# 0xC0000054/pdn-jpegxl

Measured on AMD Instinct MI355X. Metric: megapixels/sec decode (4K lossy VarDCT), higher is better.
Workload: dtype f32

## Files before the change

### pdn_jpegxl_amd/csrc/tile_kernels.hip

```cpp
#include <hip/hip_runtime.h>
#include <cstdlib>
#include "dev_types.h"
#include "dev_util.h"
#include "kernels.h"

namespace jxlhip {

#ifndef JXLHIP_PRIO_PIXEL
#define JXLHIP_PRIO_PIXEL 0
#endif
#if JXLHIP_PRIO_PIXEL
#define JXL_PIXEL_PRIO() __builtin_amdgcn_s_setprio(JXLHIP_PRIO_PIXEL)
#else
#define JXL_PIXEL_PRIO() ((void)0)
#endif

namespace {

constexpr int kTS = 64;
constexpr int kLP = 65;

__device__ const uint8_t t_quant_table[kNumStrategies] = {0, 1, 2, 3, 4, 5, 6, 6, 7, 7, 8, 8, 9, 9, 10, 10, 10, 10, 11, 12, 12, 13, 14, 14, 15, 16, 16};

__device__ __forceinline__ bool Special(uint32_t s) { return (s >= 1 && s <= 3) || (s >= 12 && s <= 17); }
typedef float __attribute__((ext_vector_type(4))) F4;
template <int N>
__device__ __forceinline__ F4 MfmaChain(const float* pa, int sa, const float* pb, int sb) {
  float a[N / 4], b[N / 4];
#pragma unroll
  for (int k = 0; k < N / 4; k++) { a[k] = pa[k * sa]; b[k] = pb[k * sb]; }
  F4 acc = {0.f, 0.f, 0.f, 0.f};
#pragma unroll
  for (int k = 0; k < N / 4; k++) acc = __builtin_amdgcn_mfma_f32_16x16x4f32(a[k], b[k], acc, 0, 0, 0);
  return acc;
}
template <bool kTableIsA>
__device__ __forceinline__ F4 MfmaChain32L(const float4* t_lo, const float4* t_hi, int pair, const float* po, int so) {
  const float4 v0 = t_lo[pair], v1 = t_hi[pair];
  const float t[8] = {v0.x, v0.y, v0.z, v0.w, v1.x, v1.y, v1.z, v1.w};
  float o[8];
#pragma unroll
  for (int k = 0; k < 8; k++) o[k] = po[k * so];
  F4 acc = {0.f, 0.f, 0.f, 0.f};
#pragma unroll
  for (int k = 0; k < 8; k++)
    acc = kTableIsA ? __builtin_amdgcn_mfma_f32_16x16x4f32(t[k], o[k], acc, 0, 0, 0) : __builtin_amdgcn_mfma_f32_16x16x4f32(o[k], t[k], acc, 0, 0, 0);
  return acc;
}
template <bool kTableIsA>
__device__ __forceinline__ F4 MfmaChain64L(const float4* t64, int pair, const float* po, int so) {
  float t[16], o[16];
#pragma unroll
  for (int j = 0; j < 4; j++) {
    const float4 v = t64[j * 256 + pair];
    t[4 * j] = v.x; t[4 * j + 1] = v.y; t[4 * j + 2] = v.z; t[4 * j + 3] = v.w;
  }
#pragma unroll
  for (int k = 0; k < 16; k++) o[k] = po[k * so];
  F4 acc = {0.f, 0.f, 0.f, 0.f};
#pragma unroll
  for (int k = 0; k < 16; k++)
    acc = kTableIsA ? __builtin_amdgcn_mfma_f32_16x16x4f32(t[k], o[k], acc, 0, 0, 0) : __builtin_amdgcn_mfma_f32_16x16x4f32(o[k], t[k], acc, 0, 0, 0);
  return acc;
}
__device__ __forceinline__ bool MfmaRows(uint32_t tl, uint32_t tr) {
  return (tl >> 31) && (tr >> 31) && ((tl >> 21) & 7) >= 1 && ((tl >> 21) & 7) == ((tr >> 21) & 7) && ((tl >> 13) & 31) == ((tr >> 13) & 31);
}
__device__ __forceinline__ bool MfmaCols(uint32_t tl, uint32_t bl) {
  return (tl >> 31) && (bl >> 31) && ((tl >> 18) & 7) >= 1 && ((tl >> 18) & 7) == ((bl >> 18) & 7) && ((tl >> 8) & 31) == ((bl >> 8) & 31);
}

__device__ __forceinline__ float SrgbOetfT(float v) {
  const float lin = 12.92f * v;
  const float cur = 1.055f * __builtin_amdgcn_exp2f(__builtin_amdgcn_logf(v) * (1.0f / 2.4f)) - 0.055f;
  return v <= 0.0031308f ? lin : cur;
}
__device__ __forceinline__ float SrgbOetf255T(float v) {
  const float lin = (12.92f * 255.0f) * v;
  const float cur = (1.055f * 255.0f) * __builtin_amdgcn_exp2f(__builtin_amdgcn_logf(v) * (1.0f / 2.4f)) - (0.055f * 255.0f);
  return v <= 0.0031308f ? lin : cur;
}
__device__ __forceinline__ float PowT(float a, float e) { return __builtin_amdgcn_exp2f(__builtin_amdgcn_logf(a) * e); }
__device__ __forceinline__ float EncodeTransferT(int kind, float v, float pq_scale, const float* lut = nullptr) {
  if (kind == 0) return v;
  if (kind == 5) {
    const float t = __builtin_sqrtf(fminf(fmaxf(v, 0.f), 1.f)) * 4095.0f;
    const int i = min((int)t, 4094);
    return lut[i] + (lut[i + 1] - lut[i]) * (t - (float)i);
  }
  const float a = fabsf(v);
  float r;
  if (kind == 1) r = a <= 0.0031308f ? 12.92f * a : 1.055f * PowT(a, 1.0f / 2.4f) - 0.055f;
  else if (kind == 2) r = a < 0.018f ? 4.5f * a : 1.099f * PowT(a, 0.45f) - 0.099f;
  else {
    const float xp = a > 0.f ? PowT(a * pq_scale, 0.1593017578125f) : 0.f;
    r = a > 0.f ? PowT((0.8359375f + 18.8515625f * xp) / (1.0f + 18.6875f * xp), 78.84375f) : 0.f;
  }
  return copysignf(r, v);
}
__device__ __forceinline__ uint8_t ToU8T(float v) {
  v = fminf(fmaxf(v * 255.0f, 0.f), 255.0f);
  return (uint8_t)(v + 0.5f);
}

__device__ __forceinline__ uint32_t LoadAlpha(const DevImage& im, size_t i) {
// ... 44 lines not shown
    }
  }
}
__device__ __forceinline__ void WritePixelA(const DevImage& im, int x, int y, float X, float Y, float B, uint32_t a) {
  WritePixelAt(im, [&] { return (size_t)(y - im.band_y0) * im.w + x; }, X, Y, B, a);
}
__device__ __forceinline__ bool PlainOutput(const DevImage& im) { return im.out_bits == 8 && im.to_srgb <= 1 && !im.unpremultiply && !im.has_noise; }
__device__ __forceinline__ float NoiseStrength(const DevImage& im, float v) {
  const float s = fmaxf(0.f, 6.0f * v);
  const int i = (int)fminf(s, 6.0f);
  const float t = fminf(s - (float)i, 1.0f);
  const float lo = im.noise_lut[i], hi = im.noise_lut[i + 1];
  return fminf(fmaxf(lo + (hi - lo) * t, 0.f), 1.0f);
}
__device__ __forceinline__ void AddNoise(const DevImage& im, int x, int y, float& X, float& Y, float& B) {
  const size_t o = (size_t)y * im.w + x;
  const float n0 = im.noise[0][o], n1 = im.noise[1][o], n2 = im.noise[2][o];
  const float sr = NoiseStrength(im, 0.5f * (Y + X)), sg = NoiseStrength(im, 0.5f * (Y - X));
  const float shared = n2 * (127.0f / 128.0f);
  const float red = (n0 * (1.0f / 128.0f) + shared) * sr, green = (n1 * (1.0f / 128.0f) + shared) * sg;
  const float rg = red + green;
  X += im.base_x * rg + (red - green);
  Y += rg;
  B += im.base_b * rg;
}
__device__ __forceinline__ uint32_t PixelToRgba8(const DevImage& im, float X, float Y, float B, uint32_t a) {
  const float gr = Y + X - im.opsin_bias_cbrt[0], gg = Y - X - im.opsin_bias_cbrt[1], gb = B - im.opsin_bias_cbrt[2];
  const float mr = gr * gr * gr + im.opsin_bias[0], mg = gg * gg * gg + im.opsin_bias[1], mb = gb * gb * gb + im.opsin_bias[2];
  float r = im.opsin_inv[0] * mr + im.opsin_inv[1] * mg + im.opsin_inv[2] * mb;
  float g = im.opsin_inv[3] * mr + im.opsin_inv[4] * mg + im.opsin_inv[5] * mb;
  float bl = im.opsin_inv[6] * mr + im.opsin_inv[7] * mg + im.opsin_inv[8] * mb;
  if (im.to_srgb) { r = SrgbOetf255T(r); g = SrgbOetf255T(g); bl = SrgbOetf255T(bl); }
  else { r *= 255.0f; g *= 255.0f; bl *= 255.0f; }
  uint32_t px = a << 24;
  px = __builtin_amdgcn_cvt_pk_u8_f32(r, 0, px);
  px = __builtin_amdgcn_cvt_pk_u8_f32(g, 1, px);
  px = __builtin_amdgcn_cvt_pk_u8_f32(bl, 2, px);
  return px;
}
__device__ __noinline__ void WritePixelGeneral(const DevImage& im, int x, int y, float X, float Y, float B, uint32_t a) {
  if (im.has_noise) {
    AddNoise(im, x, y, X, Y, B);
    if (im.out_bits == 8 && im.to_srgb <= 1 && !im.unpremultiply && im.final_stage == 5 &&
        (im.noise_pairs_twin || (im.nch_out == 4 && (x | 3) < im.w))) {
      const uint32_t px = PixelToRgba8(im, X, Y, B, a);
      uint8_t* out = im.out + ((size_t)(y - im.band_y0) * im.w + x) * im.nch_out;
      if (im.nch_out == 4) *(uint32_t*)out = px;
      else if (im.nch_out == 3) { out[0] = (uint8_t)px; out[1] = (uint8_t)(px >> 8); out[2] = (uint8_t)(px >> 16); }
      else { out[0] = (uint8_t)(px >> 8); if (im.nch_out == 2) out[1] = (uint8_t)(px >> 24); }
      return;
    }
  }
  WritePixelA(im, x, y, X, Y, B, a);
}
__device__ __forceinline__ void WritePixel(const DevImage& im, int x, int y, float X, float Y, float B) {
  const uint32_t a = im.has_alpha ? LoadAlpha(im, (size_t)y * im.w + x) : 0u;
  if (im.has_noise) { WritePixelGeneral(im, x, y, X, Y, B, a); return; }
  WritePixelA(im, x, y, X, Y, B, a);
}

}

#define JXL_IDCT_STEP(Bp, v0, v1)                                                                  \
  {                                                                                                \
    const float4 b0 = *(const float4*)(Bp);                                                        \
    const float4 b1 = *(const float4*)((Bp) + 4);                                                  \
    a0[0] += v0 * b0.x; a0[1] += v0 * b0.y; a0[2] += v0 * b0.z; a0[3] += v0 * b0.w;                \
    a0[4] += v0 * b1.x; a0[5] += v0 * b1.y; a0[6] += v0 * b1.z; a0[7] += v0 * b1.w;                \
    a1[0] += v1 * b0.x; a1[1] += v1 * b0.y; a1[2] += v1 * b0.z; a1[3] += v1 * b0.w;                \
    a1[4] += v1 * b1.x; a1[5] += v1 * b1.y; a1[6] += v1 * b1.z; a1[7] += v1 * b1.w;                \
  }

__device__ __forceinline__ float DequantBias(int32_t v, float qb, float qb3) {
  if (v == 0) return 0.f;
  if (v == 1) return qb;
  if (v == -1) return -qb;
  const float f = (float)v;
  return f - qb3 * __builtin_amdgcn_rcpf(f);
}
typedef int __attribute__((ext_vector_type(4))) I4v;

constexpr int kTileF = kTS * kLP;

__global__ __launch_bounds__(768, 6) void recon_tile_kernel(const DevImage* __restrict__ imgs, const float* basis_all, const float* basis_small,
                                                             const float* llf_scale, const float* basis_mfma) {
  JXL_PIXEL_PRIO();
  extern __shared__ __align__(16) uint8_t smem_raw[];
  float* cfc3 = (float*)smem_raw;
  float* B816 = cfc3 + 3 * kTileF;
  float* cscale = B816 + 320;
  uint32_t* ci = (uint32_t*)(cscale + 64);
  uint32_t* cmeta = ci + 64;
  uint32_t* cnq = cmeta + 64;
  uint32_t* cpre = cnq + 64;
  uint32_t* cstart = cpre + 3 * 64;
  uint32_t* ctot = cstart + 3 * 64;
  const U32x2** csc = (const U32x2**)(ctot + 4);
  float4* t32_lo = (float4*)(csc + 64);
  float4* t32_hi = t32_lo + 128;
  float4* t64 = t32_hi + 128;
  const DevImage& im = imgs[blockIdx.y];
  const int tile = blockIdx.x;
  if (tile >= im.wt * im.ht) return;
  const int tid = threadIdx.x;
  const int tx = tile % im.wt, ty = tile / im.wt;
  if (ty < im.dec_gy0 * 4 || ty >= im.dec_gy1 * 4) return;
  const int wave = tid >> 6, lane = tid & 63, team = wave >> 2, tw = wave & 3;
  const int c = team == 0 ? 1 : (team == 1 ? 0 : 2);
  const int wp = im.wp, hp = im.hp;
  {
    float4* z = (float4*)cfc3;
    for (int i = tid; i < 3 * kTileF / 4; i += 768) z[i] = make_float4(0.f, 0.f, 0.f, 0.f);
  }
  int bad = 0, has64 = 0;
  if (tid < 64) {
    const int cx = tx * 8 + (tid & 7), cy = ty * 8 + (tid >> 3);
    const bool inside = cx < im.w8 && cy < im.h8;
    const size_t cell_g = (size_t)min(cy, im.h8 - 1) * im.w8 + min(cx, im.w8 - 1);
    const size_t ncells = (size_t)im.w8 * im.h8;
    const uint32_t info_g = im.cellinfo[cell_g];
    const uint32_t rq_g = im.rawq[cell_g];
    U32x2 blk[3];
    blk[0] = im.cblk[ncells + cell_g]; blk[1] = im.cblk[cell_g]; blk[2] = im.cblk[2 * ncells + cell_g];
    const uint32_t info = inside ? info_g : 0u;
    const uint32_t rqv = inside ? rq_g : 1u;
    const int ix = (info >> 8) & 31, iy = (info >> 13) & 31, lcx = (info >> 18) & 7, lcy = (info >> 21) & 7;
    if (inside) {
      if (!(info >> 31)) bad = 1;
      else {
        const int ox = (tid & 7) - ix, oy = (tid >> 3) - iy;
        bad = ox < 0 || oy < 0 || ox + (1 << lcx) > 8 || oy + (1 << lcy) > 8 || Special(info & 0xFF) ||
              (ox & ((1 << lcx) - 1)) != 0 || (oy & ((1 << lcy) - 1)) != 0;
      }
    }
    const bool valid = (info >> 31) && !bad;
    has64 = valid && (lcx == 3 || lcy == 3);
    {
      const uint64_t any = __ballot(has64);
      if (tid == 0) ctot[3] = any != 0;
    }
    const uint32_t q = t_quant_table[valid ? (info & 0xFF) : 0];
    const uint32_t rq_origin = (uint32_t)__shfl((int)rqv, valid ? tid - iy * 8 - ix : tid);
    const uint32_t lng = 3 + max(lcx, lcy);
    const bool transposed = lcy >= lcx;
    ci[tid] = info;
    cscale[tid] = im.inv_global_scale / (float)rq_origin;
    cmeta[tid] = lng | (transposed ? 16u : 0u);
    cnq[tid] = im.dq_n[q];
    csc[tid] = im.scan[q];
    const bool origin = valid && ix == 0 && iy == 0;
    uint32_t cnt[3], sum[3];
#pragma unroll
    for (int t = 0; t < 3; t++) {
      cnt[t] = origin ? blk[t].y : 0u;
      if (cnt[t] > 65536u || blk[t].x > kGroupEntriesCap - cnt[t]) cnt[t] = 0;
      sum[t] = cnt[t];
    }
#pragma unroll
    for (int d = 1; d < 64; d <<= 1) {
#pragma unroll
      for (int t = 0; t < 3; t++) {
        const uint32_t a = (uint32_t)__shfl_up((int)sum[t], d);
        if (tid >= d) sum[t] += a;
      }
    }
#pragma unroll
    for (int t = 0; t < 3; t++) {
      cpre[t * 64 + tid] = sum[t] - cnt[t];
      cstart[t * 64 + tid] = blk[t].x;
      if (tid == 63) ctot[t] = sum[t];
    }
  } else if (tid < 64 + 320) {
    B816[tid - 64] = basis_all[tid - 64];
  } else if (tid < 64 + 320 + 256) {
    const int i = tid - (64 + 320);
    const float4 v = ((const float4*)basis_mfma)[i];
    if (i & 1) t32_hi[i >> 1] = v; else t32_lo[i >> 1] = v;
  }
  if (im.num_passes > 1) bad = 1;
  if (__syncthreads_or(bad)) {
    if (tid == 0) im.tile_list[atomicAdd(&im.status[1], 1u)] = (uint32_t)tile;
    return;
  }
  if (ctot[3]) {
    for (int i = tid; i < 1024; i += 768) t64[(i & 3) * 256 + (i >> 2)] = ((const float4*)(basis_mfma + 1024))[i];
  }
  const float* const Bl = basis_all;
  float* const cfc = cfc3 + team * kTileF;
  if (tw == 0) {
    const int cxg = tx * 8 + (lane & 7), cyg = ty * 8 + (lane >> 3);
    const bool inside = cxg < im.w8 && cyg < im.h8;
    const float lf_g = im.lf_final[c][(size_t)min(cyg, im.h8 - 1) * im.w8 + min(cxg, im.w8 - 1)];
    const float lfv = inside ? lf_g : 0.f;
    const uint32_t info = ci[lane];
    const bool valid = info >> 31;
    const int ix = (info >> 8) & 31, iy = (info >> 13) & 31, lcx = (info >> 18) & 7, lcy = (info >> 21) & 7;
    const int cx = 1 << lcx, cy = 1 << lcy;
    const int ox = (lane & 7) - ix, oy = (lane >> 3) - iy;
    const float* Bx = basis_small + (cx * cx - 1) / 3 + ix * cx;
    const float* By = basis_small + (cy * cy - 1) / 3 + iy * cy;
    float bx[8], byv[8];
#pragma unroll
    for (int k = 0; k < 8; k++) { bx[k] = (valid && k < cx) ? Bx[k] : 0.f; byv[k] = (valid && k < cy) ? By[k] : 0.f; }
    const float sc = valid ? llf_scale[lcy * 32 + iy] * llf_scale[lcx * 32 + ix] / (float)(cx * cy) : 0.f;
    float row = 0.f;
#pragma unroll
    for (int k = 0; k < 8; k++) {
      const float v = __shfl(lfv, (lane - ix + k) & 63);
      if (valid && k < cx) row += v * bx[k];
    }
    float acc = 0.f;
#pragma unroll
    for (int k = 0; k < 8; k++) {
      const float v = __shfl(row, ((oy + k) * 8 + (lane & 7)) & 63);
      if (valid && k < cy) acc += v * byv[k];
    }
    if (valid) atomicAdd(&cfc[(oy * 8 + iy) * kLP + ox * 8 + ix], acc * sc);
  }
  {
    const size_t tile_cfl = (size_t)ty * im.wt + tx;
    const float cfl_x = im.base_x + (float)im.ytox[tile_cfl] * im.inv_color_factor;
    const float cfl_b = im.base_b + (float)im.ytob[tile_cfl] * im.inv_color_factor;
    const uint32_t* entries = im.centries + (size_t)((ty >> 2) * im.xg + (tx >> 2) - im.centries_g0) * kGroupEntriesCap;
    const uint32_t t0 = ctot[0], t01 = t0 + ctot[1], total = t01 + ctot[2];
    const float qb3 = im.qbias[3];
    for (uint32_t e = (uint32_t)tid; e < total; e += 768) {
      const uint32_t t = (e >= t0) + (e >= t01);
      const uint32_t el = e - (t == 0 ? 0u : (t == 1 ? t0 : t01));
      const uint32_t* pre = cpre + t * 64;
      uint32_t j = 0;
#pragma unroll
      for (int step = 32; step; step >>= 1) if (pre[j + step] <= el) j += step;
      const uint32_t ent = entries[cstart[t * 64 + j] + (el - pre[j])];
      const uint32_t k = ent & 0xFFFFu, nq = cnq[j];
      if (k >= nq) continue;
      const int chan = t == 0 ? 1 : (t == 1 ? 0 : 2);
      const U32x2 se = csc[j][(size_t)chan * nq + k];
      const uint32_t meta = cmeta[j];
      const uint32_t lng = meta & 15, p = se.x;
      const uint32_t r = p >> lng, cc = p & ((1u << lng) - 1);
      const uint32_t ky = (meta & 16) ? cc : r, kx = (meta & 16) ? r : cc;
      if (ky >= 64 || kx >= 64) continue;
      const int32_t v = (int32_t)ent >> 16;
      const float dm = t == 0 ? 1.0f : (t == 1 ? im.x_dm : im.b_dm);
      const float o = DequantBias(v, im.qbias[chan], qb3) * (cscale[j] * dm) * __uint_as_float(se.y);
      const uint32_t at = ((j >> 3) * 8 + ky) * kLP + (j & 7) * 8 + kx;
      atomicAdd(&cfc3[t * kTileF + at], o);
      if (t == 0) {
        if (cfl_x != 0.f) atomicAdd(&cfc3[kTileF + at], o * cfl_x);
        if (cfl_b != 0.f) atomicAdd(&cfc3[2 * kTileF + at], o * cfl_b);
      }
    }
  }
  __syncthreads();
  const int l16 = tid & 15, lq = lane >> 4;
  {
    F4 acc[4];
    bool m[4];
    const int x0 = tw * 16;
#pragma unroll
    for (int rb = 0; rb < 4; rb++) {
      const uint32_t inf = ci[rb * 16 + tw * 2];
      m[rb] = MfmaRows(inf, ci[rb * 16 + tw * 2 + 1]);
      if (m[rb]) {
        const int iy = (inf >> 13) & 31, lcy = (inf >> 21) & 7, R = 8 << lcy;
        const float* cp = cfc + ((rb * 2 - iy) * 8 + lq) * kLP + x0 + l16;
        if (R == 16) acc[rb] = MfmaChain<16>(B816 + 64 + lq * 16 + iy * 8 + l16, 64, cp, 4 * kLP);
        else if (R == 32) acc[rb] = MfmaChain32L<true>(t32_lo, t32_hi, (iy * 8 + l16) * 4 + lq, cp, 4 * kLP);
        else acc[rb] = MfmaChain64L<true>(t64, (iy * 8 + l16) * 4 + lq, cp, 4 * kLP);
      }
    }
    const int x = x0 + (lane & 7) * 2, cr = lane >> 3;
    const uint32_t info = ci[cr * 8 + (x >> 3)];
    const bool valu = (info >> 31) && !MfmaRows(ci[(cr >> 1) * 16 + (x >> 4) * 2], ci[(cr >> 1) * 16 + (x >> 4) * 2 + 1]);
    float a0[8] = {0, 0, 0, 0, 0, 0, 0, 0}, a1[8] = {0, 0, 0, 0, 0, 0, 0, 0};
    if (valu) {
      const int iy = (info >> 13) & 31, lcy = (info >> 21) & 7;
      const int R = 8 << lcy;
      const float* in = cfc + (cr - iy) * 8 * kLP + x;
      if (R == 8) {
#pragma unroll 2
        for (int k = 0; k < 8; k++) { const float v0 = in[k * kLP], v1 = in[k * kLP + 1]; JXL_IDCT_STEP(B816 + k * 8, v0, v1) }
      } else if (R == 16) {
        const float* B = B816 + 64 + iy * 8;
#pragma unroll 2
        for (int k = 0; k < 16; k++) { const float v0 = in[k * kLP], v1 = in[k * kLP + 1]; JXL_IDCT_STEP(B + k * 16, v0, v1) }
      } else {
        const float* B = Bl + (R * R - 64) / 3 + iy * 8;
        for (int k = 0; k < R; k++) { const float v0 = in[k * kLP], v1 = in[k * kLP + 1]; JXL_IDCT_STEP(B + k * R, v0, v1) }
      }
    }
    __builtin_amdgcn_fence(__ATOMIC_RELEASE, "wavefront");
    __builtin_amdgcn_wave_barrier();
#pragma unroll
    for (int rb = 0; rb < 4; rb++)
      if (m[rb]) {
        float* o = cfc + (rb * 16 + 4 * lq) * kLP + x0 + l16;
        o[0] = acc[rb].x; o[kLP] = acc[rb].y; o[2 * kLP] = acc[rb].z; o[3 * kLP] = acc[rb].w;
      }
    if (valu) {
#pragma unroll
      for (int j = 0; j < 8; j++) { cfc[(cr * 8 + j) * kLP + x] = a0[j]; cfc[(cr * 8 + j) * kLP + x + 1] = a1[j]; }
    }
  }
  __syncthreads();
  {
    F4 acc[4];
    bool m[4];
    const int y0 = tw * 16;
#pragma unroll
    for (int cs = 0; cs < 4; cs++) {
      const uint32_t inf = ci[tw * 16 + cs * 2];
      m[cs] = MfmaCols(inf, ci[tw * 16 + 8 + cs * 2]);
      if (m[cs]) {
        const int ix = (inf >> 8) & 31, lcx = (inf >> 18) & 7, C = 8 << lcx;
        const float* ap = cfc + (y0 + l16) * kLP + (cs * 2 - ix) * 8 + lq;
        if (C == 16) acc[cs] = MfmaChain<16>(ap, 4, B816 + 64 + lq * 16 + ix * 8 + l16, 64);
        else if (C == 32) acc[cs] = MfmaChain32L<false>(t32_lo, t32_hi, (ix * 8 + l16) * 4 + lq, ap, 4);
        else acc[cs] = MfmaChain64L<false>(t64, (ix * 8 + l16) * 4 + lq, ap, 4);
      }
    }
    const int y = y0 + (lane & 7) * 2, cc = lane >> 3;
    const uint32_t info = ci[(y >> 3) * 8 + cc];
    const bool valu = (info >> 31) && !MfmaCols(ci[(y >> 4) * 16 + (cc >> 1) * 2], ci[(y >> 4) * 16 + 8 + (cc >> 1) * 2]);
    float a0[8] = {0, 0, 0, 0, 0, 0, 0, 0}, a1[8] = {0, 0, 0, 0, 0, 0, 0, 0};
    if (valu) {
      const int ix = (info >> 8) & 31, lcx = (info >> 18) & 7;
      const int C = 8 << lcx;
      const float* in = cfc + y * kLP + (cc - ix) * 8;
      if (C == 8) {
#pragma unroll 2
        for (int k = 0; k < 8; k++) { const float v0 = in[k], v1 = in[k + kLP]; JXL_IDCT_STEP(B816 + k * 8, v0, v1) }
      } else if (C == 16) {
        const float* B = B816 + 64 + ix * 8;
#pragma unroll 2
        for (int k = 0; k < 16; k++) { const float v0 = in[k], v1 = in[k + kLP]; JXL_IDCT_STEP(B + k * 16, v0, v1) }
      } else {
        const float* B = Bl + (C * C - 64) / 3 + ix * 8;
        for (int k = 0; k < C; k++) { const float v0 = in[k], v1 = in[k + kLP]; JXL_IDCT_STEP(B + k * C, v0, v1) }
      }
    }
    __builtin_amdgcn_fence(__ATOMIC_RELEASE, "wavefront");
    __builtin_amdgcn_wave_barrier();
#pragma unroll
    for (int cs = 0; cs < 4; cs++)
      if (m[cs]) {
        float* o = cfc + (y0 + 4 * lq) * kLP + cs * 16 + l16;
        o[0] = acc[cs].x; o[kLP] = acc[cs].y; o[2 * kLP] = acc[cs].z; o[3 * kLP] = acc[cs].w;
      }
    if (valu) {
#pragma unroll
      for (int j = 0; j < 8; j++) { cfc[y * kLP + cc * 8 + j] = a0[j]; cfc[(y + 1) * kLP + cc * 8 + j] = a1[j]; }
    }
    __builtin_amdgcn_fence(__ATOMIC_ACQ_REL, "wavefront");
    __builtin_amdgcn_wave_barrier();
    float* dst = im.xyb[c];
    const int x4 = l16 * 4;
    const int gx = tx * kTS + x4;
#pragma unroll
    for (int it = 0; it < 4; it++) {
      const int yl = y0 + lq + 4 * it;
      const int gy = ty * kTS + yl;
      const float* r = cfc + yl * kLP + x4;
      const float4 o = make_float4(r[0], r[1], r[2], r[3]);
      if (gx < wp && gy < hp) *(float4*)(dst + (size_t)gy * wp + gx) = o;
    }
  }
}

template <int kStage>
__global__ __launch_bounds__(256) void filter_tile_kernel(const DevImage* __restrict__ imgs) {
  JXL_PIXEL_PRIO();
  constexpr int TW = 64, TH = 32;
  constexpr int HALO = kStage == 0 ? 1 : (kStage == 1 ? 3 : (kStage == 2 ? 2 : 1));
  constexpr int LW = TW + 2 * HALO, LH = TH + 2 * HALO;
  __shared__ float t[3][LH][LW + 1];
  const DevImage& im = imgs[blockIdx.y];
  if (!im.stage_on[kStage]) return;
  const int w = im.w, h = im.h, wp = im.wp;
  const int tiles_x = (w + TW - 1) / TW, tiles_y = (h + TH - 1) / TH;
  if ((int)blockIdx.x >= tiles_x * tiles_y) return;
  const int tx = blockIdx.x % tiles_x, ty = blockIdx.x / tiles_x;
  const int x0 = tx * TW, y0 = ty * TH;
  const bool final_stage = im.final_stage == kStage;
  const int row_lo = final_stage ? im.band_y0 : max(0, im.band_y0 - 8), row_hi = final_stage ? im.band_y1 : min(h, im.band_y1 + 8);
  if (y0 + TH <= row_lo || y0 >= row_hi) return;
  const float* in0 = im.stage_in[kStage][0];
  const float* in1 = im.stage_in[kStage][1];
  const float* in2 = im.stage_in[kStage][2];
  constexpr int kLoadIters = (LW * LH + 255) / 256;
#pragma unroll
  for (int it = 0; it < kLoadIters; it++) {
    const int e0 = threadIdx.x + it * 256;
    const int e = e0 < LW * LH ? e0 : LW * LH - 1;
    const int ly = e / LW, lx = e % LW;
    const size_t g = (size_t)ReflectIndex(y0 - HALO + ly, h) * wp + ReflectIndex(x0 - HALO + lx, w);
    const float v0 = in0[g], v1 = in1[g], v2 = in2[g];
    t[0][ly][lx] = v0;
    t[1][ly][lx] = v1;
    t[2][ly][lx] = v2;
  }
  __syncthreads();
#pragma unroll 2
  for (int e = threadIdx.x; e < TW * TH; e += 256) {
    const int ly = e / TW, lx = e % TW;
    const int x = x0 + lx, y = y0 + ly;
    if (x >= w || y < row_lo || y >= row_hi) continue;
    const int cy = ly + HALO, cx = lx + HALO;
    float o0, o1, o2;
    if (kStage == 0) {
      float o[3];
#pragma unroll
      for (int c = 0; c < 3; c++) {
        o[c] = t[c][cy][cx] * im.gab_w[c][0] +
               (t[c][cy - 1][cx] + t[c][cy + 1][cx] + t[c][cy][cx - 1] + t[c][cy][cx + 1]) * im.gab_w[c][1] +
               (t[c][cy - 1][cx - 1] + t[c][cy - 1][cx + 1] + t[c][cy + 1][cx - 1] + t[c][cy + 1][cx + 1]) * im.gab_w[c][2];
      }
      o0 = o[0]; o1 = o[1]; o2 = o[2];
    } else {
      constexpr int kNoff = kStage == 1 ? 12 : 4;
      constexpr int kNplus = kStage == 3 ? 1 : 5;
      const int off0[12][2] = {{-2, 0}, {-1, -1}, {-1, 0}, {-1, 1}, {0, -2}, {0, -1}, {0, 1}, {0, 2}, {1, -1}, {1, 0}, {1, 1}, {2, 0}};
      const int off1[4][2] = {{-1, 0}, {0, -1}, {0, 1}, {1, 0}};
      const int plus[5][2] = {{0, 0}, {-1, 0}, {1, 0}, {0, -1}, {0, 1}};
      const float is = im.inv_sigma[(size_t)(y >> 3) * im.w8 + (x >> 3)];
      o0 = t[0][cy][cx]; o1 = t[1][cy][cx]; o2 = t[2][cy][cx];
      if (!(is < -3.90524291751269967465540850526868f)) {
        const float sm = kStage == 1 ? im.epf_pass0_sigma_scale : (kStage == 2 ? 1.0f : im.epf_pass2_sigma_scale);
        const bool border = ((x & 7) == 0) || ((x & 7) == 7) || ((y & 7) == 0) || ((y & 7) == 7);
        const float inv = is * (border ? sm * im.epf_border_sad_mul : sm);
        float wsum = 1.0f;
#pragma unroll
        for (int k = 0; k < kNoff; k++) {
          const int dy = kStage == 1 ? off0[k][0] : off1[k][0], dx = kStage == 1 ? off0[k][1] : off1[k][1];
          float s0 = 0.f, s1 = 0.f, s2 = 0.f;
#pragma unroll
          for (int p = 0; p < kNplus; p++) {
            const int ay = cy + plus[p][0], ax = cx + plus[p][1];
            s0 += fabsf(t[0][ay][ax] - t[0][ay + dy][ax + dx]);
            s1 += fabsf(t[1][ay][ax] - t[1][ay + dy][ax + dx]);
            s2 += fabsf(t[2][ay][ax] - t[2][ay + dy][ax + dx]);
          }
          const float sad = s0 * im.epf_channel_scale[0] + s1 * im.epf_channel_scale[1] + s2 * im.epf_channel_scale[2];
          const float wt = fmaxf(0.0f, 1.0f + sad * inv);
          wsum += wt;
          o0 += wt * t[0][cy + dy][cx + dx];
          o1 += wt * t[1][cy + dy][cx + dx];
          o2 += wt * t[2][cy + dy][cx + dx];
        }
        const float iw = 1.0f / wsum;
        o0 *= iw; o1 *= iw; o2 *= iw;
      }
    }
    if (final_stage) {
      WritePixel(im, x, y, o0, o1, o2);
    } else {
      const size_t g = (size_t)y * wp + x;
      im.stage_out[kStage][0][g] = o0;
      im.stage_out[kStage][1][g] = o1;
      im.stage_out[kStage][2][g] = o2;
    }
  }
}

constexpr int kStripLanes = 64;
constexpr int kStripOut = 4 * (kStripLanes - 2);
constexpr int kGroupsPerWg = 256 / kStripLanes;
constexpr int kSegRows = 128;
__device__ __forceinline__ float DppFromLeft(float v) {
  return __builtin_bit_cast(float, __builtin_amdgcn_update_dpp(0, __builtin_bit_cast(int, v), 0x138 , 0xF, 0xF, true));
}
__device__ __forceinline__ float DppFromRight(float v) {
  return __builtin_bit_cast(float, __builtin_amdgcn_update_dpp(0, __builtin_bit_cast(int, v), 0x130 , 0xF, 0xF, true));
}
__device__ __forceinline__ F4 ShiftFromLeft(F4 v) { return F4{DppFromLeft(v.w), v.x, v.y, v.z}; }
__device__ __forceinline__ F4 ShiftFromRight(F4 v) { return F4{v.y, v.z, v.w, DppFromRight(v.x)}; }
__device__ __forceinline__ F4 ShiftFromLeft2(F4 v) { return F4{DppFromLeft(v.z), DppFromLeft(v.w), v.x, v.y}; }
__device__ __forceinline__ F4 Abs(F4 v) { return F4{fabsf(v.x), fabsf(v.y), fabsf(v.z), fabsf(v.w)}; }
typedef float __attribute__((ext_vector_type(2))) F2;
typedef unsigned __attribute__((ext_vector_type(2))) U2v;
__device__ __forceinline__ F2 ShiftFromLeft(F2 v) { return F2{DppFromLeft(v.y), v.x}; }
__device__ __forceinline__ F2 ShiftFromRight(F2 v) { return F2{v.y, DppFromRight(v.x)}; }
__device__ __forceinline__ F2 ShiftFromLeft2(F2 v) { return F2{DppFromLeft(v.x), DppFromLeft(v.y)}; }
__device__ __forceinline__ F2 Abs(F2 v) { return F2{fabsf(v.x), fabsf(v.y)}; }

template <typename V> struct RowOf { V c[3]; };
template <typename V> constexpr int kLanePixels = sizeof(V) / sizeof(float);
typedef RowOf<F4> Row3;
typedef RowOf<F2> PairRow;
#define JXL_GLOBAL __attribute__((address_space(1)))
__device__ __forceinline__ Row3 LoadRow3(const JXL_GLOBAL float* p0, const JXL_GLOBAL float* p1, const JXL_GLOBAL float* p2, int X, int y, int w, int h,
                                         int wp, bool interior) {
  const int yy = ReflectIndex(y, h);
  Row3 r;
  if (interior) {
    const size_t g = (size_t)yy * wp + X;
    r.c[0] = *(const JXL_GLOBAL F4*)(p0 + g); r.c[1] = *(const JXL_GLOBAL F4*)(p1 + g); r.c[2] = *(const JXL_GLOBAL F4*)(p2 + g);
  } else {
    const size_t g = (size_t)yy * wp;
    const int x0 = ReflectIndex(X, w), x1 = ReflectIndex(X + 1, w), x2 = ReflectIndex(X + 2, w), x3 = ReflectIndex(X + 3, w);
    r.c[0] = F4{p0[g + x0], p0[g + x1], p0[g + x2], p0[g + x3]};
    r.c[1] = F4{p1[g + x0], p1[g + x1], p1[g + x2], p1[g + x3]};
    r.c[2] = F4{p2[g + x0], p2[g + x1], p2[g + x2], p2[g + x3]};
  }
  return r;
}
template <typename V> struct Windows {
  RowOf<V> in[4], s[4], g[4];
  V dv[4], dh[4], hd[4];
};
typedef Windows<F4> StreamState;
typedef Windows<F2> PairState;
template <typename V>
__device__ __forceinline__ void ZeroWindows(Windows<V>& st) {
  const V zero = V(0.f);
#pragma unroll
  for (int i = 0; i < 4; i++) {
#pragma unroll
    for (int c = 0; c < 3; c++) { st.in[i].c[c] = zero; st.s[i].c[c] = zero; st.g[i].c[c] = zero; }
    st.dv[i] = zero; st.dh[i] = zero; st.hd[i] = zero;
  }
}
struct RowConst {
  float gw0[3], gw1[3], gw2[3], cs[3], bsm;
  int y0, y1;
};
__device__ __forceinline__ void FillRowConst(const DevImage& im, RowConst& k) {
  const bool no_gab = im.stream_no_gab != 0;
#pragma unroll
  for (int c = 0; c < 3; c++) {
    k.gw0[c] = no_gab ? 1.0f : im.gab_w[c][0]; k.gw1[c] = no_gab ? 0.0f : im.gab_w[c][1]; k.gw2[c] = no_gab ? 0.0f : im.gab_w[c][2];
    k.cs[c] = im.epf_channel_scale[c];
  }
  k.bsm = im.epf_border_sad_mul;
}
template <typename V>
__device__ __forceinline__ V BorderInv(float inv_in, float inv_b, bool xb_first, bool xb_last) {
  V inv = V(inv_in);
  inv[0] = xb_first ? inv_b : inv_in; inv[kLanePixels<V> - 1] = xb_last ? inv_b : inv_in;
  return inv;
}

template <int P, typename V>
__device__ __forceinline__ bool GabEpf1Row(const RowOf<V>& cur, Windows<V>& st, const RowConst& k, float is, int y, bool xb_first, bool xb_last,
                                           V o[3]) {
  constexpr int s0 = P, s1 = (P + 1) & 3, s2 = (P + 2) & 3, s3 = (P + 3) & 3;
  const V zero = V(0.f);
  V dhn = zero, dvn = zero;
  st.in[s0] = cur;
#pragma unroll
  for (int c = 0; c < 3; c++) {
    st.s[s0].c[c] = ShiftFromLeft(cur.c[c]) + ShiftFromRight(cur.c[c]);
    const V gn = st.in[s3].c[c] * k.gw0[c] + ((st.in[s2].c[c] + cur.c[c]) + st.s[s3].c[c]) * k.gw1[c] + (st.s[s2].c[c] + st.s[s0].c[c]) * k.gw2[c];
    dhn += Abs(gn - ShiftFromRight(gn)) * k.cs[c];
    dvn += Abs(st.g[s2].c[c] - gn) * k.cs[c];
    st.g[s3].c[c] = gn;
  }
  const V dv0 = st.dv[s3], dv1 = st.dv[s0], dv2 = st.dv[s1];
  const V hd2 = ShiftFromLeft(dv2) + ShiftFromRight(dv2);
  const V hd1 = st.hd[s0];
  const bool output_row = y >= k.y0 && y < k.y1;
  if (output_row) {
    const V dh0 = st.dh[s0], dh1 = st.dh[s1], dh2 = st.dh[s2];
    const V a = dv1 + dv2;
    const V sad_u = a + dv0 + hd1, sad_d = a + dvn + hd2;
    const V vh = dh0 + dh1 + dh2;
    const V sad_r = vh + (ShiftFromLeft(dh1) + ShiftFromRight(dh1));
    const V sad_l = ShiftFromLeft(vh) + (ShiftFromLeft2(dh1) + dh1);
    const bool yb = ((y & 7) == 0) || ((y & 7) == 7);
    const V inv = BorderInv<V>(is * (yb ? k.bsm : 1.0f), is * k.bsm, xb_first, xb_last);
    const bool skip = is < -3.90524291751269967465540850526868f;
    V wu, wl, wr, wd, iw;
#pragma unroll
// ... 409 lines not shown
  k.out = PlaneResource(im.out);
  const float cs[3] = {im.epf_channel_scale[0], im.epf_channel_scale[1], im.epf_channel_scale[2]};
  const float sm = im.epf_pass2_sigma_scale, smb = sm * im.epf_border_sad_mul;
  PairRow prev = LoadPairRow(k, k.y0 - 1);
  PairRow cur = LoadPairRow(k, k.y0);
  PairRow next = LoadPairRow(k, min(k.y0 + 1, k.r_end - 1));
  PairAux aux = LoadPairAux(k, k.y0);
  for (int y = k.y0; y < k.y1; y++) {
    const PairRow next2 = LoadPairRow(k, min(y + 2, k.r_end - 1));
    const PairAux aux2 = LoadPairAux(k, y + 1);
    const uint32_t al = k.use_alpha ? aux.al : 0xFFFFu;
    F2 o[3];
    Epf2Row(prev, cur, next, cs, sm, smb, aux.is, y, k.xb_lo, k.xb_hi, o);
    if (k.stores) {
      StorePixelPair(k, PixelToRgba8(im, o[0].x, o[1].x, o[2].x, al & 0xFF), PixelToRgba8(im, o[0].y, o[1].y, o[2].y, (al >> 8) & 0xFF), y - k.band_y0);
    }
    prev = cur; cur = next; next = next2; aux = aux2;
  }
}

__global__ void out_only_kernel(const DevImage* __restrict__ imgs) {
  const DevImage& im = imgs[blockIdx.y];
  if (im.final_stage != 4) return;
  const int w = im.w, wp = im.wp;
  const size_t n = (size_t)w * (im.band_y1 - im.band_y0);
  for (size_t i = (size_t)blockIdx.x * blockDim.x + threadIdx.x; i < n; i += (size_t)gridDim.x * blockDim.x) {
    const int x = (int)(i % w), y = im.band_y0 + (int)(i / w);
    const size_t o = (size_t)y * wp + x;
    WritePixel(im, x, y, im.stage_in[4][0][o], im.stage_in[4][1][o], im.stage_in[4][2][o]);
  }
}

__device__ __forceinline__ void LfOutputPixel(const DevImage& im, size_t i, float X, float Y, float B) {
  const int cx = (int)(i % (size_t)im.ds_w), cy = (int)(i / (size_t)im.ds_w);
  const size_t o = OrientedIndex(im.ds_orient, cx, cy, im.ds_w, im.ds_h);
  const uint32_t a = !im.has_alpha ? 0u : (im.out_bits == 8 ? (uint32_t)im.ds_alpha[i] : (im.out_bits == 16 ? (uint32_t)((const uint16_t*)im.ds_alpha)[i]
                                                                                                              : ((const uint32_t*)im.ds_alpha)[i]));
  if (PlainOutput(im)) {
    const uint32_t px = PixelToRgba8(im, X, Y, B, a);
    uint8_t* out = im.out + o * im.nch_out;
    if (im.nch_out == 4) *(uint32_t*)out = px;
    else if (im.nch_out == 3) { out[0] = (uint8_t)px; out[1] = (uint8_t)(px >> 8); out[2] = (uint8_t)(px >> 16); }
    else { out[0] = (uint8_t)(px >> 8); if (im.nch_out == 2) out[1] = (uint8_t)(px >> 24); }
    return;
  }
  WritePixelAt(im, [&] { return o; }, X, Y, B, a);
}
__global__ __launch_bounds__(256) void lf_output_kernel(const DevImage* __restrict__ imgs) {
  const DevImage& im = imgs[blockIdx.y];
  if (!im.ds || im.is_modular) return;
  const size_t n = (size_t)im.ds_w * im.ds_h;
  const float* __restrict__ pX = im.lf_final[0];
  const float* __restrict__ pY = im.lf_final[1];
  const float* __restrict__ pB = im.lf_final[2];
  const size_t gid = (size_t)blockIdx.x * blockDim.x + threadIdx.x, stride = (size_t)gridDim.x * blockDim.x;
  const bool quads = PlainOutput(im) && im.ds_orient == 1 && im.ncolor == 3 && ((uintptr_t)im.out & 15) == 0;
  if (!quads) {
    for (size_t i = gid; i < n; i += stride) LfOutputPixel(im, i, pX[i], pY[i], pB[i]);
    return;
  }
  const size_t nq = n >> 2;
  for (size_t q = gid; q < nq; q += stride) {
    const float4 X = ((const float4*)pX)[q], Y = ((const float4*)pY)[q], B = ((const float4*)pB)[q];
    const uint32_t a = im.has_alpha ? ((const uint32_t*)im.ds_alpha)[q] : 0u;
    const uint32_t p0 = PixelToRgba8(im, X.x, Y.x, B.x, a & 0xFF), p1 = PixelToRgba8(im, X.y, Y.y, B.y, (a >> 8) & 0xFF);
    const uint32_t p2 = PixelToRgba8(im, X.z, Y.z, B.z, (a >> 16) & 0xFF), p3 = PixelToRgba8(im, X.w, Y.w, B.w, a >> 24);
    if (im.nch_out == 4) ((uint4*)im.out)[q] = make_uint4(p0, p1, p2, p3);
    else ((uint3*)im.out)[q] = make_uint3((p0 & 0xFFFFFFu) | (p1 << 24), ((p1 >> 8) & 0xFFFFu) | (p2 << 16), ((p2 >> 16) & 0xFFu) | (p3 << 8));
  }
  if (blockIdx.x == 0 && threadIdx.x < (n & 3)) {
    const size_t i = 4 * nq + threadIdx.x;
    LfOutputPixel(im, i, pX[i], pY[i], pB[i]);
  }
}

void LaunchLfOutput(const DevImage* imgs, int nimg, size_t max_cells, hipStream_t s) {
  if (nimg <= 0) return;
  const size_t b = std::min<size_t>((max_cells + 255) / 256, 2048);
  hipLaunchKernelGGL(lf_output_kernel, dim3((unsigned)std::max<size_t>(1, b), nimg), dim3(256), 0, s, imgs);
}

void LaunchReconTiles(const DevImage* imgs, int nimg, int max_tiles, const float* basis_all, const float* basis_small,
                      const float* llf_scale, const float* basis_mfma, hipStream_t s) {
  const size_t lds = (size_t)(3 * kTileF + 320 + 64 * 4 + 64 * 6 + 4 + 128 + 1024 + 4096) * 4;
  static bool raised = false;
  if (!raised) { (void)hipFuncSetAttribute((const void*)recon_tile_kernel, hipFuncAttributeMaxDynamicSharedMemorySize, (int)lds); raised = true; }
  hipLaunchKernelGGL(recon_tile_kernel, dim3(max_tiles, nimg), dim3(768), lds, s, imgs, basis_all, basis_small, llf_scale, basis_mfma);
}

void LaunchFilterTiles(const DevImage* imgs, int nimg, int max_w, int max_h, int stage_mask, bool any_unfiltered,
                       int any_fused, int any_fused2, hipStream_t s) {
  const int tiles = ((max_w + 63) / 64) * ((max_h + 31) / 32);
  dim3 g(tiles, nimg);
  if (stage_mask & 1) hipLaunchKernelGGL(filter_tile_kernel<0>, g, dim3(256), 0, s, imgs);
  if (stage_mask & 2) hipLaunchKernelGGL(filter_tile_kernel<1>, g, dim3(256), 0, s, imgs);
  if (any_fused) {
    const int groups = ((max_w + kStripOut - 1) / kStripOut) * ((max_h + 2 + kSegRows - 1) / kSegRows);
    const int pair_groups = ((max_w + kPairOut - 1) / kPairOut) * ((max_h + 2 + kSegRows - 1) / kSegRows);
    if (any_fused & 1) hipLaunchKernelGGL(filter_stream_pairs_kernel, dim3((pair_groups + kGroupsPerWg - 1) / kGroupsPerWg, nimg), dim3(256), 0, s, imgs);
    if (any_fused & 2) hipLaunchKernelGGL(filter_stream_kernel, dim3((groups + kGroupsPerWg - 1) / kGroupsPerWg, nimg), dim3(256), 0, s, imgs);
    const int pair2_groups = ((max_w + kPair2Out - 1) / kPair2Out) * ((max_h + kSegRows - 1) / kSegRows);
    if (any_fused2 & 1) hipLaunchKernelGGL(filter_stream2_pairs_kernel, dim3((pair2_groups + kGroupsPerWg - 1) / kGroupsPerWg, nimg), dim3(256), 0, s, imgs);
    if (any_fused2 & 2) hipLaunchKernelGGL(filter_stream2_kernel, dim3((groups + kGroupsPerWg - 1) / kGroupsPerWg, nimg), dim3(256), 0, s, imgs);
  }
  if (stage_mask & 4) hipLaunchKernelGGL(filter_tile_kernel<2>, g, dim3(256), 0, s, imgs);
  if (stage_mask & 8) hipLaunchKernelGGL(filter_tile_kernel<3>, g, dim3(256), 0, s, imgs);
  if (any_unfiltered) {
    size_t work = (size_t)max_w * max_h;
    size_t b = std::min<size_t>((work + 255) / 256, 8192);
    hipLaunchKernelGGL(out_only_kernel, dim3((unsigned)b, nimg), dim3(256), 0, s, imgs);
  }
}

}
```

Baseline: 32940.

## Restructure recon tile prologue: hoist global loads, stage LLF tables in LDS, overlap fills

Reorganizes the recon_tile_kernel prologue. Image fields are hoisted into scalar registers. The LF, CFL and table loads are issued before the LDS zero-fill so their latency overlaps it. The quant-table lookup is replaced with a constexpr popcount, and the dq_n and scan lookups become lane shuffles. The LLF basis and scale tables are staged into LDS by the otherwise idle waves. The 64-point MFMA table load moves after the barrier and overlaps the coefficient scatter loop. LDS use grows slightly and register pressure rises from the hoisted values and prefetched float4s.

```diff
diff --git a/pdn_jpegxl_amd/csrc/tile_kernels.hip b/pdn_jpegxl_amd/csrc/tile_kernels.hip
--- a/pdn_jpegxl_amd/csrc/tile_kernels.hip
+++ b/pdn_jpegxl_amd/csrc/tile_kernels.hip
@@ -20,7 +20,23 @@
 constexpr int kTS = 64;
 constexpr int kLP = 65;
 
-__device__ const uint8_t t_quant_table[kNumStrategies] = {0, 1, 2, 3, 4, 5, 6, 6, 7, 7, 8, 8, 9, 9, 10, 10, 10, 10, 11, 12, 12, 13, 14, 14, 15, 16, 16};
+#define JXL_GLOBAL __attribute__((address_space(1)))
+template <class T> __device__ __forceinline__ JXL_GLOBAL T* G(T* p) { return (JXL_GLOBAL T*)p; }
+typedef unsigned __attribute__((ext_vector_type(2))) U2v;
+
+constexpr uint8_t kQuantTable[kNumStrategies] = {0, 1, 2, 3, 4, 5, 6, 6, 7, 7, 8, 8, 9, 9, 10, 10, 10, 10, 11, 12, 12, 13, 14, 14, 15, 16, 16};
+constexpr uint32_t QuantTableSteps() {
+  uint32_t m = 0;
+  for (int s = 1; s < kNumStrategies; s++) m |= (uint32_t)(kQuantTable[s] - kQuantTable[s - 1]) << s;
+  return m;
+}
+constexpr uint32_t kQuantTableSteps = QuantTableSteps();
+constexpr uint32_t QuantTableOf(uint32_t strategy) { return (uint32_t)__builtin_popcount(kQuantTableSteps & ((2u << (strategy & 31)) - 1u)); }
+constexpr bool QuantTableIsItsSteps() {
+  for (int s = 0; s < kNumStrategies; s++) if (QuantTableOf(s) != kQuantTable[s]) return false;
+  return true;
+}
+static_assert(kNumStrategies <= 32 && QuantTableIsItsSteps(), "kQuantTable must start at 0 and step by 0 or 1");
 
 __device__ __forceinline__ bool Special(uint32_t s) { return (s >= 1 && s <= 3) || (s >= 12 && s <= 17); }
 typedef float __attribute__((ext_vector_type(4))) F4;
@@ -231,46 +247,100 @@
 
 constexpr int kTileF = kTS * kLP;
 
+struct ReconLds {
+  static constexpr int kLlfBasisWords = 88;
+  static constexpr int kLlfScaleWords = 4 * 32;
+  static constexpr int kCfc = 0;
+  static constexpr int kB816 = kCfc + 3 * kTileF;
+  static constexpr int kLlfBasis = kB816 + 320;
+  static constexpr int kLlfScale = kLlfBasis + kLlfBasisWords;
+  static constexpr int kCscale = kLlfScale + kLlfScaleWords;
+  static constexpr int kCi = kCscale + 64;
+  static constexpr int kCmeta = kCi + 64;
+  static constexpr int kCnq = kCmeta + 64;
+  static constexpr int kCpre = kCnq + 64;
+  static constexpr int kCstart = kCpre + 3 * 64;
+  static constexpr int kCtot = kCstart + 3 * 64;
+  static constexpr int kCsc = kCtot + 4;
+  static constexpr int kT32Lo = kCsc + 2 * 64;
+  static constexpr int kT32Hi = kT32Lo + 4 * 128;
+  static constexpr int kT64 = kT32Hi + 4 * 128;
+  static constexpr int kWords = kT64 + 4 * 1024;
+  static constexpr size_t kBytes = (size_t)kWords * 4;
+};
+static_assert(ReconLds::kCsc % 2 == 0 && ReconLds::kT32Lo % 4 == 0 && ReconLds::kLlfBasis % 4 == 0, "pointers at 8, float4 tables at 16 bytes");
+static_assert(ReconLds::kBytes <= 80 * 1024, "two workgroups of recon_tile_kernel per compute unit");
+
 __global__ __launch_bounds__(768, 6) void recon_tile_kernel(const DevImage* __restrict__ imgs, const float* basis_all, const float* basis_small,
                                                              const float* llf_scale, const float* basis_mfma) {
   JXL_PIXEL_PRIO();
   extern __shared__ __align__(16) uint8_t smem_raw[];
-  float* cfc3 = (float*)smem_raw;
-  float* B816 = cfc3 + 3 * kTileF;
-  float* cscale = B816 + 320;
-  uint32_t* ci = (uint32_t*)(cscale + 64);
-  uint32_t* cmeta = ci + 64;
-  uint32_t* cnq = cmeta + 64;
-  uint32_t* cpre = cnq + 64;
-  uint32_t* cstart = cpre + 3 * 64;
-  uint32_t* ctot = cstart + 3 * 64;
-  const U32x2** csc = (const U32x2**)(ctot + 4);
-  float4* t32_lo = (float4*)(csc + 64);
-  float4* t32_hi = t32_lo + 128;
-  float4* t64 = t32_hi + 128;
+  float* const smem = (float*)smem_raw;
+  float* cfc3 = smem + ReconLds::kCfc;
+  float* B816 = smem + ReconLds::kB816;
+  const float* llf_basis = smem + ReconLds::kLlfBasis;
+  const float* llf_sc = smem + ReconLds::kLlfScale;
+  float* cscale = smem + ReconLds::kCscale;
+  uint32_t* ci = (uint32_t*)(smem + ReconLds::kCi);
+  uint32_t* cmeta = (uint32_t*)(smem + ReconLds::kCmeta);
+  uint32_t* cnq = (uint32_t*)(smem + ReconLds::kCnq);
+  uint32_t* cpre = (uint32_t*)(smem + ReconLds::kCpre);
+  uint32_t* cstart = (uint32_t*)(smem + ReconLds::kCstart);
+  uint32_t* ctot = (uint32_t*)(smem + ReconLds::kCtot);
+  const U32x2** csc = (const U32x2**)(smem + ReconLds::kCsc);
+  float4* t32_lo = (float4*)(smem + ReconLds::kT32Lo);
+  float4* t32_hi = (float4*)(smem + ReconLds::kT32Hi);
+  float4* t64 = (float4*)(smem + ReconLds::kT64);
   const DevImage& im = imgs[blockIdx.y];
   const int tile = blockIdx.x;
-  if (tile >= im.wt * im.ht) return;
+  const int wt = im.wt, ht = im.ht, w8 = im.w8, h8 = im.h8, wp = im.wp, hp = im.hp, gy0 = im.dec_gy0, gy1 = im.dec_gy1;
+  const int xg = im.xg, centries_g0 = im.centries_g0, num_passes = im.num_passes;
+  const float inv_global_scale = im.inv_global_scale, base_x = im.base_x, base_b = im.base_b, inv_color_factor = im.inv_color_factor;
+  const float qb_x = im.qbias[0], qb_y = im.qbias[1], qb_b = im.qbias[2], qb3 = im.qbias[3], x_dm = im.x_dm, b_dm = im.b_dm;
+  const uint32_t* const f_centries = im.centries;
+  const uint32_t* const f_cellinfo = im.cellinfo;
+  const uint16_t* const f_rawq = im.rawq;
+  const U32x2* const f_cblk = im.cblk;
+  const int8_t* const f_ytox = im.ytox;
+  const int8_t* const f_ytob = im.ytob;
+  const float* const f_lf0 = im.lf_final[0];
+  const float* const f_lf1 = im.lf_final[1];
+  const float* const f_lf2 = im.lf_final[2];
+  float* const f_xyb0 = im.xyb[0];
+  float* const f_xyb1 = im.xyb[1];
+  float* const f_xyb2 = im.xyb[2];
+  asm volatile("" ::"s"(f_cellinfo), "s"(f_rawq), "s"(f_cblk), "s"(f_centries), "s"(xg), "s"(centries_g0), "s"(num_passes), "s"(inv_global_scale));
+  asm volatile("" ::"s"(basis_all), "s"(basis_small), "s"(llf_scale), "s"(basis_mfma), "s"(f_xyb0), "s"(f_xyb1), "s"(f_xyb2));
+  asm volatile("" ::"s"(base_x), "s"(base_b), "s"(inv_color_factor), "s"(qb_x), "s"(qb_y), "s"(qb_b), "s"(qb3), "s"(x_dm), "s"(b_dm));
+  if (tile >= wt * ht) return;
   const int tid = threadIdx.x;
-  const int tx = tile % im.wt, ty = tile / im.wt;
-  if (ty < im.dec_gy0 * 4 || ty >= im.dec_gy1 * 4) return;
-  const int wave = tid >> 6, lane = tid & 63, team = wave >> 2, tw = wave & 3;
+  const int tx = tile % wt, ty = tile / wt;
+  if (ty < gy0 * 4 || ty >= gy1 * 4) return;
+  const int wave = __builtin_amdgcn_readfirstlane(tid >> 6), lane = tid & 63, team = wave >> 2, tw = wave & 3;
   const int c = team == 0 ? 1 : (team == 1 ? 0 : 2);
-  const int wp = im.wp, hp = im.hp;
-  {
+  const int cell_x = tx * 8 + (lane & 7), cell_y = ty * 8 + (lane >> 3);
+  const bool cell_inside = cell_x < w8 && cell_y < h8;
+  const size_t cell_g = (size_t)min(cell_y, h8 - 1) * w8 + min(cell_x, w8 - 1);
+  float lf_g = 0.f;
+  if (tw == 0) lf_g = G(c == 1 ? f_lf1 : (c == 0 ? f_lf0 : f_lf2))[cell_g];
+  const size_t tile_cfl = (size_t)ty * wt + tx;
+  const int ytox = G(f_ytox)[tile_cfl], ytob = G(f_ytob)[tile_cfl];
+  const auto zero_fill = [&] {
     float4* z = (float4*)cfc3;
     for (int i = tid; i < 3 * kTileF / 4; i += 768) z[i] = make_float4(0.f, 0.f, 0.f, 0.f);
-  }
-  int bad = 0, has64 = 0;
-  if (tid < 64) {
-    const int cx = tx * 8 + (tid & 7), cy = ty * 8 + (tid >> 3);
-    const bool inside = cx < im.w8 && cy < im.h8;
-    const size_t cell_g = (size_t)min(cy, im.h8 - 1) * im.w8 + min(cx, im.w8 - 1);
-    const size_t ncells = (size_t)im.w8 * im.h8;
-    const uint32_t info_g = im.cellinfo[cell_g];
-    const uint32_t rq_g = im.rawq[cell_g];
-    U32x2 blk[3];
-    blk[0] = im.cblk[ncells + cell_g]; blk[1] = im.cblk[cell_g]; blk[2] = im.cblk[2 * ncells + cell_g];
+  };
+  int bad = 0;
+  if (wave == 0) {
+    const size_t ncells = (size_t)w8 * h8;
+    const JXL_GLOBAL U2v* cblk = (const JXL_GLOBAL U2v*)f_cblk;
+    const uint32_t info_g = G(f_cellinfo)[cell_g];
+    const uint32_t rq_g = G(f_rawq)[cell_g];
+    const U2v blk[3] = {cblk[ncells + cell_g], cblk[cell_g], cblk[2 * ncells + cell_g]};
+    const int ql = lane < kNumQuantTables ? lane : 0;
+    const uint32_t dqn_l = ((const JXL_GLOBAL uint32_t*)im.dq_n)[ql];
+    const U32x2* const scan_l = ((const U32x2* const JXL_GLOBAL*)im.scan)[ql];
+    zero_fill();
+    const bool inside = cell_inside;
     const uint32_t info = inside ? info_g : 0u;
     const uint32_t rqv = inside ? rq_g : 1u;
     const int ix = (info >> 8) & 31, iy = (info >> 13) & 31, lcx = (info >> 18) & 7, lcy = (info >> 21) & 7;
@@ -283,20 +353,24 @@
       }
     }
     const bool valid = (info >> 31) && !bad;
-    has64 = valid && (lcx == 3 || lcy == 3);
+    const int has64 = valid && (lcx == 3 || lcy == 3);
     {
       const uint64_t any = __ballot(has64);
       if (tid == 0) ctot[3] = any != 0;
     }
-    const uint32_t q = t_quant_table[valid ? (info & 0xFF) : 0];
+    const uint32_t q = QuantTableOf(valid ? (info & 0xFF) : 0);
     const uint32_t rq_origin = (uint32_t)__shfl((int)rqv, valid ? tid - iy * 8 - ix : tid);
     const uint32_t lng = 3 + max(lcx, lcy);
     const bool transposed = lcy >= lcx;
     ci[tid] = info;
-    cscale[tid] = im.inv_global_scale / (float)rq_origin;
+    cscale[tid] = inv_global_scale / (float)rq_origin;
     cmeta[tid] = lng | (transposed ? 16u : 0u);
-    cnq[tid] = im.dq_n[q];
-    csc[tid] = im.scan[q];
+    cnq[tid] = (uint32_t)__shfl((int)dqn_l, (int)q);
+    {
+      const uint64_t sp = (uint64_t)scan_l;
+      const uint32_t lo = (uint32_t)__shfl((int)(uint32_t)sp, (int)q), hi = (uint32_t)__shfl((int)(uint32_t)(sp >> 32), (int)q);
+      csc[tid] = (const U32x2*)(((uint64_t)hi << 32) | lo);
+    }
     const bool origin = valid && ix == 0 && iy == 0;
     uint32_t cnt[3], sum[3];
 #pragma unroll
@@ -319,39 +393,42 @@
       cstart[t * 64 + tid] = blk[t].x;
       if (tid == 63) ctot[t] = sum[t];
     }
-  } else if (tid < 64 + 320) {
-    B816[tid - 64] = basis_all[tid - 64];
-  } else if (tid < 64 + 320 + 256) {
+  } else if (wave < 6) {
+    const float v = basis_all[tid - 64];
+    zero_fill();
+    B816[tid - 64] = v;
+  } else if (wave < 10) {
     const int i = tid - (64 + 320);
     const float4 v = ((const float4*)basis_mfma)[i];
-    if (i & 1) t32_hi[i >> 1] = v; else t32_lo[i >> 1] = v;
-  }
-  if (im.num_passes > 1) bad = 1;
+    zero_fill();
+    (i & 1 ? t32_hi : t32_lo)[i >> 1] = v;
+  } else {
+    const int i = tid - (64 + 320 + 256);
+    const float b = basis_small[min(i, 84)], sc = llf_scale[i];
+    zero_fill();
+    smem[ReconLds::kLlfBasis + min(i, ReconLds::kLlfBasisWords - 1)] = b;
+    smem[ReconLds::kLlfScale + i] = sc;
+  }
+  if (num_passes > 1) bad = 1;
   if (__syncthreads_or(bad)) {
     if (tid == 0) im.tile_list[atomicAdd(&im.status[1], 1u)] = (uint32_t)tile;
     return;
   }
-  if (ctot[3]) {
-    for (int i = tid; i < 1024; i += 768) t64[(i & 3) * 256 + (i >> 2)] = ((const float4*)(basis_mfma + 1024))[i];
-  }
   const float* const Bl = basis_all;
   float* const cfc = cfc3 + team * kTileF;
   if (tw == 0) {
-    const int cxg = tx * 8 + (lane & 7), cyg = ty * 8 + (lane >> 3);
-    const bool inside = cxg < im.w8 && cyg < im.h8;
-    const float lf_g = im.lf_final[c][(size_t)min(cyg, im.h8 - 1) * im.w8 + min(cxg, im.w8 - 1)];
-    const float lfv = inside ? lf_g : 0.f;
+    const float lfv = cell_inside ? lf_g : 0.f;
     const uint32_t info = ci[lane];
     const bool valid = info >> 31;
     const int ix = (info >> 8) & 31, iy = (info >> 13) & 31, lcx = (info >> 18) & 7, lcy = (info >> 21) & 7;
     const int cx = 1 << lcx, cy = 1 << lcy;
     const int ox = (lane & 7) - ix, oy = (lane >> 3) - iy;
-    const float* Bx = basis_small + (cx * cx - 1) / 3 + ix * cx;
-    const float* By = basis_small + (cy * cy - 1) / 3 + iy * cy;
+    const float* Bx = llf_basis + (cx * cx - 1) / 3 + ix * cx;
+    const float* By = llf_basis + (cy * cy - 1) / 3 + iy * cy;
     float bx[8], byv[8];
 #pragma unroll
     for (int k = 0; k < 8; k++) { bx[k] = (valid && k < cx) ? Bx[k] : 0.f; byv[k] = (valid && k < cy) ? By[k] : 0.f; }
-    const float sc = valid ? llf_scale[lcy * 32 + iy] * llf_scale[lcx * 32 + ix] / (float)(cx * cy) : 0.f;
+    const float sc = valid ? llf_sc[lcy * 32 + iy] * llf_sc[lcx * 32 + ix] / (float)(cx * cy) : 0.f;
     float row = 0.f;
 #pragma unroll
     for (int k = 0; k < 8; k++) {
@@ -366,13 +443,15 @@
     }
     if (valid) atomicAdd(&cfc[(oy * 8 + iy) * kLP + ox * 8 + ix], acc * sc);
   }
+  const bool stage64 = ctot[3] != 0;
+  const int i64 = 768 + (tid & 255);
+  float4 v64a = make_float4(0.f, 0.f, 0.f, 0.f), v64b = v64a;
   {
-    const size_t tile_cfl = (size_t)ty * im.wt + tx;
-    const float cfl_x = im.base_x + (float)im.ytox[tile_cfl] * im.inv_color_factor;
-    const float cfl_b = im.base_b + (float)im.ytob[tile_cfl] * im.inv_color_factor;
-    const uint32_t* entries = im.centries + (size_t)((ty >> 2) * im.xg + (tx >> 2) - im.centries_g0) * kGroupEntriesCap;
+    const float cfl_x = base_x + (float)ytox * inv_color_factor;
+    const float cfl_b = base_b + (float)ytob * inv_color_factor;
+    const JXL_GLOBAL uint32_t* entries = G(f_centries) + (size_t)((ty >> 2) * xg + (tx >> 2) - centries_g0) * kGroupEntriesCap;
     const uint32_t t0 = ctot[0], t01 = t0 + ctot[1], total = t01 + ctot[2];
-    const float qb3 = im.qbias[3];
+    if (stage64) { v64a = ((const float4*)(basis_mfma + 1024))[tid]; v64b = ((const float4*)(basis_mfma + 1024))[i64]; }
     for (uint32_t e = (uint32_t)tid; e < total; e += 768) {
       const uint32_t t = (e >= t0) + (e >= t01);
       const uint32_t el = e - (t == 0 ? 0u : (t == 1 ? t0 : t01));
@@ -384,15 +463,16 @@
       const uint32_t k = ent & 0xFFFFu, nq = cnq[j];
       if (k >= nq) continue;
       const int chan = t == 0 ? 1 : (t == 1 ? 0 : 2);
-      const U32x2 se = csc[j][(size_t)chan * nq + k];
+      const U2v se = ((const JXL_GLOBAL U2v*)csc[j])[(size_t)chan * nq + k];
       const uint32_t meta = cmeta[j];
       const uint32_t lng = meta & 15, p = se.x;
       const uint32_t r = p >> lng, cc = p & ((1u << lng) - 1);
       const uint32_t ky = (meta & 16) ? cc : r, kx = (meta & 16) ? r : cc;
       if (ky >= 64 || kx >= 64) continue;
       const int32_t v = (int32_t)ent >> 16;
-      const float dm = t == 0 ? 1.0f : (t == 1 ? im.x_dm : im.b_dm);
-      const float o = DequantBias(v, im.qbias[chan], qb3) * (cscale[j] * dm) * __uint_as_float(se.y);
+      const float dm = t == 0 ? 1.0f : (t == 1 ? x_dm : b_dm);
+      const float qb = t == 0 ? qb_y : (t == 1 ? qb_x : qb_b);
+      const float o = DequantBias(v, qb, qb3) * (cscale[j] * dm) * __uint_as_float(se.y);
       const uint32_t at = ((j >> 3) * 8 + ky) * kLP + (j & 7) * 8 + kx;
       atomicAdd(&cfc3[t * kTileF + at], o);
       if (t == 0) {
@@ -401,6 +481,7 @@
       }
     }
   }
+  if (stage64) { t64[(tid & 3) * 256 + (tid >> 2)] = v64a; t64[(i64 & 3) * 256 + (i64 >> 2)] = v64b; }
   __syncthreads();
   const int l16 = tid & 15, lq = lane >> 4;
   {
@@ -503,7 +584,7 @@
     }
     __builtin_amdgcn_fence(__ATOMIC_ACQ_REL, "wavefront");
     __builtin_amdgcn_wave_barrier();
-    float* dst = im.xyb[c];
+    float* dst = c == 1 ? f_xyb1 : (c == 0 ? f_xyb0 : f_xyb2);
     const int x4 = l16 * 4;
     const int gx = tx * kTS + x4;
 #pragma unroll
@@ -627,7 +708,6 @@
 __device__ __forceinline__ F4 ShiftFromLeft2(F4 v) { return F4{DppFromLeft(v.z), DppFromLeft(v.w), v.x, v.y}; }
 __device__ __forceinline__ F4 Abs(F4 v) { return F4{fabsf(v.x), fabsf(v.y), fabsf(v.z), fabsf(v.w)}; }
 typedef float __attribute__((ext_vector_type(2))) F2;
-typedef unsigned __attribute__((ext_vector_type(2))) U2v;
 __device__ __forceinline__ F2 ShiftFromLeft(F2 v) { return F2{DppFromLeft(v.y), v.x}; }
 __device__ __forceinline__ F2 ShiftFromRight(F2 v) { return F2{v.y, DppFromRight(v.x)}; }
 __device__ __forceinline__ F2 ShiftFromLeft2(F2 v) { return F2{DppFromLeft(v.x), DppFromLeft(v.y)}; }
@@ -637,7 +717,6 @@
 template <typename V> constexpr int kLanePixels = sizeof(V) / sizeof(float);
 typedef RowOf<F4> Row3;
 typedef RowOf<F2> PairRow;
-#define JXL_GLOBAL __attribute__((address_space(1)))
 __device__ __forceinline__ Row3 LoadRow3(const JXL_GLOBAL float* p0, const JXL_GLOBAL float* p1, const JXL_GLOBAL float* p2, int X, int y, int w, int h,
                                          int wp, bool interior) {
   const int yy = ReflectIndex(y, h);
@@ -1213,7 +1292,7 @@
 
 void LaunchReconTiles(const DevImage* imgs, int nimg, int max_tiles, const float* basis_all, const float* basis_small,
                       const float* llf_scale, const float* basis_mfma, hipStream_t s) {
-  const size_t lds = (size_t)(3 * kTileF + 320 + 64 * 4 + 64 * 6 + 4 + 128 + 1024 + 4096) * 4;
+  const size_t lds = ReconLds::kBytes;
   static bool raised = false;
   if (!raised) { (void)hipFuncSetAttribute((const void*)recon_tile_kernel, hipFuncAttributeMaxDynamicSharedMemorySize, (int)lds); raised = true; }
   hipLaunchKernelGGL(recon_tile_kernel, dim3(max_tiles, nimg), dim3(768), lds, s, imgs, basis_all, basis_small, llf_scale, basis_mfma);
```

After: 33270 (median of 2 runs). No clear change (+1.0%).
